# ignaschuemer7/soft-actor-critic

Measured on AMD Instinct MI355X. Metric: SAC gradient steps/sec + replay-sample GB/s, BipedalWalker batch=256, higher is better.
Workload: dtype fp32; 1 GPU; c2: BipedalWalker-v3 obs=24 act=4 2x[256, 256] MLPs, buffer=1000000, batch=256, auto-alpha, device sampler, fp32 arithmetic; global_batch=256, parallelism=replicas1, graph_chunk=64

## Files before the change

soft-actor-critic_amd/csrc/sac_split.h:

```cpp
#pragma once
#include "sac_phases.h"

#define SPLIT_H 256
#define SPLIT_HH 128
__host__ __device__ constexpr int split_wc(int elem_bytes) { return elem_bytes == 4 ? 4 : 2; }
__host__ __device__ constexpr int split_wcq(int elem_bytes) { return (void)elem_bytes, 4; }
__host__ __device__ constexpr int split_wpi(int elem_bytes) { return split_wc(elem_bytes); }
#define SPLIT_GP 4

enum SplitGran {
  GS_PI = 0,
  GS_PS = 1,
  GS_QT1 = 2,
  GS_QT2 = 3,
  GS_LP = 4,
  GS_QA1 = 5,
  GS_QA2 = 6,
  GS_C1 = 7,
  GS_C2 = 8,
  GS_COUNT = 9
};
__device__ __forceinline__ AS_G uint64_t* gs_at(const AS_C EngineDev& E, int kind, int rbi, int h) {
  return GP(uint64_t, E.gran2) + ((size_t)(kind * E.nrt + rbi) * SPLIT_GP + h) * E.gs2;
}

template <typename T, int NTW, int HC>
struct HTiles {
  typename MM<T>::Frag f[NTW][HC];
  float b[NTW];
};

template <typename T, int NTW, int HC, bool COH = false>
__device__ __forceinline__ void ht_issue(HTiles<T, NTW, HC>& ht, const GemmW& w) {
  constexpr uint32_t FSB = 64 * MM<T>::KL * sizeof(T);
  const int lane = threadIdx.x & 63, wave = wave_id();
  const int nch = w.cols / MM<T>::KC;
  const __amdgpu_buffer_rsrc_t rs = coh_rsrc(w.p, 0xFFFFFFF0u);
  static_for<NTW>([&](auto jc) {
    constexpr int j = decltype(jc)::value;
    int t = wave + j * SAC_NW;
    const bool has = t < w.NT;
    t = has ? t : w.NT - 1;
    const uint32_t o = (uint32_t)(((size_t)t * 16 * w.tcols + lane * MM<T>::KL) * sizeof(T));
    static_for<HC>([&](auto uc) {
      constexpr int u = decltype(uc)::value;
      const uint32_t cu = u < nch ? u : nch - 1;
      if (has)
        ht.f[j][u] = coh_frag<T, COH>(rs, o + cu * FSB);
      else
        ht.f[j][u] = typename MM<T>::Frag{};
    });
    if (w.bias) {
      const int n = t * 16 + (lane & 15);
      ht.b[j] = ldf<COH>(w.bias + (n < w.N ? n : w.N - 1));
    }
  });
}

template <typename T, int NTW, int HC, bool COH = false, typename Epi>
__device__ __forceinline__ void gemm_hs(const lf* __restrict__ A, int lda, const GemmW& w,
                                        const HTiles<T, NTW, HC>* ht, Epi&& epi) {
  typedef typename MM<T>::Frag F;
  constexpr int KC = MM<T>::KC, KL = MM<T>::KL;
  constexpr uint32_t FSB = 64 * KL * sizeof(T);
  const int lane = threadIdx.x & 63, wave = wave_id();
  const int c = lane & 15, g = lane >> 4;
  const int nch = w.cols / KC;
  const lf* arow = A + c * lda + g * KL;
  f32x4 acc[NTW][2];
  static_for<NTW>([&](auto jc) {
    constexpr int j = decltype(jc)::value;
    acc[j][0] = acc[j][1] = (f32x4){0.f, 0.f, 0.f, 0.f};
  });
  int ch0 = 0;
  if (ht) {
    F a[HC];
    static_for<HC>([&](auto uc) {
      constexpr int u = decltype(uc)::value;
      a[u] = MM<T>::from_lds(arow + (u < nch ? u : 0) * KC);
    });
    static_for<HC>([&](auto uc) {
      constexpr int u = decltype(uc)::value;
      if (u < nch)
        static_for<NTW>([&](auto jc) {
          constexpr int j = decltype(jc)::value;
          if (wave + j * SAC_NW < w.NT)
            MM<T>::mma(acc[j][u & 1], a[u], ht->f[j][u]);
        });
    });
    ch0 = HC;
  }
  if (ch0 < nch) {
    const __amdgpu_buffer_rsrc_t rs = coh_rsrc(w.p, 0xFFFFFFF0u);
    uint32_t o[NTW];
    static_for<NTW>([&](auto jc) {
      constexpr int j = decltype(jc)::value;
      int t = wave + j * SAC_NW;
      t = t < w.NT ? t : w.NT - 1;
      o[j] = (uint32_t)(((size_t)t * 16 * w.tcols + lane * KL) * sizeof(T));
    });
    for (int cb = ch0; cb < nch; cb += 8) {
      const int rem = nch - cb < 8 ? nch - cb : 8;
      F f[NTW][8], a[8];
      static_for<8>([&](auto uc) {
        constexpr int u = decltype(uc)::value;
        const uint32_t cu = cb + (u < rem ? u : rem - 1);
        static_for<NTW>([&](auto jc) {
          constexpr int j = decltype(jc)::value;
          f[j][u] = coh_frag<T, COH>(rs, o[j] + cu * FSB);
        });
      });
      static_for<8>([&](auto uc) {
        constexpr int u = decltype(uc)::value;
        a[u] = MM<T>::from_lds(arow + (cb + (u < rem ? u : rem - 1)) * KC);
      });
      static_for<8>([&](auto uc) {
        constexpr int u = decltype(uc)::value;
        if (u < rem)
          static_for<NTW>([&](auto jc) {
            constexpr int j = decltype(jc)::value;
            if (wave + j * SAC_NW < w.NT) MM<T>::mma(acc[j][u & 1], a[u], f[j][u]);
          });
      });
    }
  }
  static_for<NTW>([&](auto jc) {
    constexpr int j = decltype(jc)::value;
    const int t = wave + j * SAC_NW;
    if (t < w.NT) epi(j, t * 16 + c, acc[j][0] + acc[j][1]);
  });
}

#ifndef SAC_KS_HELD
#define SAC_KS_HELD 1
#endif
#ifndef SAC_KS_MAXC32
#define SAC_KS_MAXC32 1
#endif
#ifndef SAC_KS_C
#define SAC_KS_C 1
#endif
template <typename T, int MC = (sizeof(T) == 4 ? SAC_KS_MAXC32 : 1)>
struct KsHeld {
  static constexpr int MAXC = MC;
  typename MM<T>::Frag f[MAXC];
  bool ok;
};
template <typename T>
__device__ __forceinline__ void ks_slice(const GemmW& w, int& t, int& c0, int& c1, int& wpt) {
  const int wave = wave_id();
  const int NT = w.NT;
  wpt = SAC_NW / NT;
  t = wave % NT;
  const int sl = wave / NT;
  const int nch = w.cols / MM<T>::KC;
  const int per = (nch + wpt - 1) / wpt;
  c0 = sl * per;
  c1 = c0 + per < nch ? c0 + per : nch;
}
template <typename T, int MC, bool COH = false>
__device__ __forceinline__ void ks_issue(KsHeld<T, MC>& kh, const GemmW& w) {
  constexpr uint32_t FSB = 64 * MM<T>::KL * sizeof(T);
  int t, c0, c1, wpt;
  ks_slice<T>(w, t, c0, c1, wpt);
  const int nch = w.cols / MM<T>::KC, per = (nch + wpt - 1) / wpt;
  kh.ok = SAC_KS_HELD && per <= MC;
  if (!kh.ok) return;
  const __amdgpu_buffer_rsrc_t rs = coh_rsrc(w.p, 0xFFFFFFF0u);
  const uint32_t o = (uint32_t)(((size_t)t * 16 * w.tcols + (threadIdx.x & 63) * MM<T>::KL) * sizeof(T));
  static_for<MC>([&](auto uc) {
    constexpr int u = decltype(uc)::value;
    if (c0 + u < c1) kh.f[u] = coh_frag<T, COH>(rs, o + (c0 + u) * FSB);
  });
}

template <typename T, bool COH = false, int MC = 1>
__device__ __forceinline__ void gemm_ksplit(const lf* __restrict__ A, int lda, const GemmW& w, lf* red, lf* out,
                                            int ldo, const KsHeld<T, MC>* kh = nullptr) {
  typedef typename MM<T>::Frag F;
  constexpr int KC = MM<T>::KC, KL = MM<T>::KL;
  constexpr uint32_t FSB = 64 * KL * sizeof(T);
  const int lane = threadIdx.x & 63, wave = wave_id();
  const int c = lane & 15, g = lane >> 4;
  const int NT = w.NT;
  int t, c0, c1, wpt;
  ks_slice<T>(w, t, c0, c1, wpt);
  const __amdgpu_buffer_rsrc_t rs = coh_rsrc(w.p, 0xFFFFFFF0u);
  const uint32_t o = (uint32_t)(((size_t)t * 16 * w.tcols + lane * KL) * sizeof(T));
  const lf* arow = A + c * lda + g * KL;
  f32x4 acc = {0.f, 0.f, 0.f, 0.f};
  if (kh && kh->ok) {
    static_for<MC>([&](auto uc) {
      constexpr int u = decltype(uc)::value;
      if (c0 + u < c1) MM<T>::mma(acc, MM<T>::from_lds(arow + (c0 + u) * KC), kh->f[u]);
    });
    c1 = c0;
  }
  for (int cb = c0; cb < c1; cb += 4) {
    const int rem = c1 - cb < 4 ? c1 - cb : 4;
    F f[4], a[4];
    static_for<4>([&](auto uc) {
      constexpr int u = decltype(uc)::value;
      const int cu = cb + (u < rem ? u : rem - 1);
      f[u] = coh_frag<T, COH>(rs, o + cu * FSB);
      a[u] = MM<T>::from_lds(arow + cu * KC);
    });
    static_for<4>([&](auto uc) {
      constexpr int u = decltype(uc)::value;
      if (u < rem) MM<T>::mma(acc, a[u], f[u]);
    });
  }
#pragma unroll
  for (int i = 0; i < 4; ++i) red[wave * 256 + (g * 4 + i) * 16 + c] = acc[i];
  __syncthreads();
  for (int i = threadIdx.x; i < 256 * NT; i += SAC_THREADS) {
    const int tt = i / 256, e = i % 256, r = e / 16, cc = e % 16;
    float s = 0.f;
    for (int q = 0; q < wpt; ++q) s += red[(q * NT + tt) * 256 + e];
    out[r * ldo + tt * 16 + cc] = s;
  }
  __syncthreads();
}

template <typename T>
__device__ __forceinline__ void target_critic_split_body(const EngineDev* __restrict__ Ep, const sac_replay& rb,
                                                         const int32_t* __restrict__ inj_idx_,
                                                         const float* __restrict__ inj_eps_, int bidA,
                                                         const StepCtx& sc) {
  const AS_C EngineDev& E = *(const AS_C EngineDev*)Ep;
  extern __shared__ float lds_raw[];
  lf* lds = (lf*)lds_raw;
  constexpr int R = SAC_ROWS, HH = SPLIT_HH;
  constexpr int KC = MM<T>::KC;
  constexpr int HC0 = 64 / KC;
  constexpr int NCH_H = SPLIT_H / KC;
  constexpr int NCH_HH = HH / KC;
  const int tid = threadIdx.x;
  constexpr int WP = split_wpi(sizeof(T));
  const int n2 = 2 * E.nrt, n0 = WP * E.nrt;
  const int grp = bidA < n0 ? 0 : 1 + (bidA - n0) / n2;
  const int idx = bidA < n0 ? bidA : (bidA - n0) % n2;
  const int h = bidA < n0 ? idx % WP : idx & 1, rbi = bidA < n0 ? idx / WP : idx >> 1;
  const int HHr = grp == 0 ? SPLIT_H / WP : SPLIT_HH;
  const int role = grp;
  const bool is_pi = role == 0 || role == 5;
  const int ni = is_pi ? NET_PI : role <= 2 ? NET_Q1T + role - 1 : NET_Q1 + role - 3;
  const AS_C NetDev& net = E.net[ni];
  const AS_C LayerDev& L0 = net.l[0];
  const AS_C LayerDev& L1 = net.l[1];
  const AS_C LayerDev& L2 = net.l[2];
  STAMP(0);
  const GemmW w0 = gw_fwd(L0);
  const GemmW w1 = gw_sub<T>(L1.Wc, L1.Kp, h * HHr, HHr, 0, L1.Kp, L1.bias + h * HHr, HHr);
  HTiles<T, 2, HC0> h0;
  HTiles<T, 1, NCH_H> h1;
  ht_issue<T, 2, HC0>(h0, w0);

  const int B = E.B, Bp = E.Bp, O = E.O, A = E.A, ld = E.ld, ldo = E.ldo;
  const int r0 = rbi * R;
  const int nvalid = min(R, B - r0);
  const uint32_t ep = sc.ep;
  const AS_G int32_t* inj_idx = GPC(int32_t, inj_idx_);
  const AS_G float* inj_eps = GPC(float, inj_eps_);
  lf* Xb = lds + E.o_X;
  lf* H0 = lds + E.o_Y;
  lf* P0 = lds + E.o_P1[0];
  lf* P1 = lds + E.o_P1[1];
  lf* H1 = lds + E.o_P2[0];
  lf* U1 = lds + E.o_P2[1];
  const int ldp0 = E.ldp1[0], ldp1 = E.ldp1[1], ldh1 = E.ldp2[0], ldu1 = E.ldp2[1];
  lf* outB = lds + E.o_out;
  lf* red = lds + E.o_red;
  lf* sB = lds + E.o_s;
  lf* s2B = lds + E.o_s2;
  lf* aB = lds + E.o_a;
  lf* a2B = lds + E.o_a2;
  lf* rB = lds + E.o_r;
  lf* dB = lds + E.o_d;
  lf* epsB = lds + E.o_et;
  lf* lpB = lds + E.o_lp;
  AS_L int64_t* slotB = (AS_L int64_t*)(lds + E.o_slot);
  AS_G float* stats = GP(float, E.stats);

  const uint64_t step = sc.step;
  const int par = sc.par;
#ifndef SAC_ADAM_LAST
#define SAC_ADAM_LAST 1
#endif
  const bool adam_blk = (SAC_ADAM_LAST ? (role == 5 && rbi == E.nrt - 1 && h == 1) : (role == 0 && rbi == 0 && h == 0));
  if (adam_blk && tid < 4 && (tid < 3 || (E.auto_entropy && E.alpha_update))) {
    const double t = GP(double, E.opt_steps)[tid] + 1.0;
    GP(double, E.opt_steps)[tid] = t;
    if (tid < 3) {
      const double lr = tid == 0 ? E.actor_lr : E.critic_lr;
      GP(float, E.adam_sc)[par * 6 + tid * 2] = (float)(-(lr / (1.0 - pow((double)E.beta1, t))));
      GP(float, E.adam_sc)[par * 6 + tid * 2 + 1] = (float)sqrt(1.0 - pow((double)E.beta2, t));
    } else {
      GP(double, E.alpha_sc)[par * 2] = 1.0 - pow((double)E.beta1, t);
      GP(double, E.alpha_sc)[par * 2 + 1] = 1.0 - pow((double)E.beta2, t);
    }
  }
  const int64_t rb_size = GPC(int64_t, rb.state)[0], rb_pos = GPC(int64_t, rb.state)[1];
  bool staged = false;
  bool h1_issued = false;
  if (E.stage && !inj_idx) {
    const AS_G float* rec = GPC(float, E.stg) + stage_rec(E, step, rbi);
    const AS_C uint64_t* hdr = (const AS_C uint64_t*)rec;
    const AS_G float* p = rec + 16;
    constexpr int NS = (R * 32 + SAC_THREADS - 1) / SAC_THREADS;
    if (O <= 32) {
      float rs[2][NS], ra[NS], rr = 0.f, rd = 0.f;
#pragma unroll
      for (int u = 0; u < NS; ++u) {
        const int i = tid + u * SAC_THREADS;
        rs[0][u] = i < R * O ? p[i] : 0.f;
        rs[1][u] = i < R * O ? p[R * O + i] : 0.f;
        ra[u] = i < R * A ? p[2 * R * O + i] : 0.f;
      }
      if (tid < R) {
        rr = p[2 * R * O + R * A + tid];
        rd = p[2 * R * O + R * A + R + tid];
      }
      ht_issue<T, 1, NCH_H>(h1, w1);
      h1_issued = true;
#pragma unroll
      for (int u = 0; u < NS; ++u) {
        const int i = tid + u * SAC_THREADS;
        if (i < R * O) {
          sB[i] = rs[0][u];
          s2B[i] = rs[1][u];
        }
        if (i < R * A) aB[i] = ra[u];
      }
      if (tid < R) {
        rB[tid] = rr;
        dB[tid] = rd;
      }
      STAMP(22);
    } else {
      for (int i = tid; i < R * O; i += SAC_THREADS) {
        sB[i] = p[i];
        s2B[i] = p[R * O + i];
      }
      for (int i = tid; i < R * A; i += SAC_THREADS) aB[i] = p[2 * R * O + i];
      if (tid < R) {
        rB[tid] = p[2 * R * O + R * A + tid];
        dB[tid] = p[2 * R * O + R * A + R + tid];
      }
    }
    staged = hdr[0] == step && hdr[1] == (uint64_t)rb_size && hdr[2] == (uint64_t)rb_pos &&
             hdr[3] == (uint64_t)(uintptr_t)rb.obs && hdr[4] == (uint64_t)GPC(int64_t, rb.state)[2];
  }
  if (!h1_issued) ht_issue<T, 1, NCH_H>(h1, w1);
  GemmW w2n = gw_sub<T>(L2.Wc, L2.Kp, 0, L2.Np, h * HHr, HHr, nullptr, 0);
  w2n.NT = (L2.N + 15) >> 4;
  KsHeld<T> kh2;
  kh2.ok = false;
  if (sizeof(T) == 2) ks_issue<T>(kh2, w2n);
  if (staged && rbi == 0 && role == 0 && h == 0 && tid == 0)
    *(AS_G uint64_t*)(GP(uint32_t, E.sync) + 4) = step;
  if (!staged) {
    tile_slots(E, rb, step, rb_size, rb_pos, r0, inj_idx, slotB);
    __syncthreads();
    gather_rows<lf*>(rb, slotB, O, A, sB, s2B, aB, rB, dB);
  }
  if (role == 1 || role == 2 || role == 5) {
    const int which = role == 5 ? 1 : 0;
    const int NP = (A + 1) / 2;
    for (int i = tid; i < R * NP; i += SAC_THREADS) {
      const int r = i / NP, pp = i % NP, b = r0 + r;
      float e0 = 0.f, e1 = 0.f;
      if (b < B) {
        if (inj_eps) {
          e0 = inj_eps[((size_t)which * B + b) * A + 2 * pp];
          if (2 * pp + 1 < A) e1 = inj_eps[((size_t)which * B + b) * A + 2 * pp + 1];
        } else {
          philox_normal2(E.seed, step, (uint32_t)b, (uint32_t)which, (uint32_t)pp, e0, e1);
        }
      }
      epsB[r * A + 2 * pp] = e0;
      if (2 * pp + 1 < A) epsB[r * A + 2 * pp + 1] = e1;
    }
  }
  __syncthreads();
  STAMP(1);

  auto head = [&](const AS_G uint64_t* g0, const AS_G uint64_t* g1, bool tgt, lf* actB, lf* lpOut, bool stash) {
    const AS_C NetDev& pn = E.net[NET_PI];
    const float* b2 = pn.l[2].bias;
    const int AP = A <= 1 ? 1 : 1 << (32 - __builtin_clz(A - 1));
    const int rpp = SAC_THREADS / AP;
    const int jj = tid % AP;
    const float b2mu = jj < A ? ldf<false>(b2 + jj) : 0.f, b2ls = jj < A ? ldf<false>(b2 + A + jj) : 0.f;
    for (int base = 0; base < R; base += rpp) {
      const int r = base + tid / AP, j = jj;
      const bool live = r < R && j < A;
      float lp = 0.f, corr = 0.f;
      if (live) {
        float mu, lsr;
        if (tgt) {
          const AS_G uint64_t* gg[2 * WP];
#pragma unroll
          for (int p = 0; p < WP; ++p) {
            gg[p] = g0 + (size_t)p * E.gs2 + r * 2 * A + j;
            gg[WP + p] = g0 + (size_t)p * E.gs2 + r * 2 * A + A + j;
          }
          float v[2 * WP];
          gran_getn<2 * WP>(E, gg, ep, v);
          float smu = v[0], sls = v[WP];
#pragma unroll
          for (int p = 1; p < WP; ++p) {
            smu += v[p];
            sls += v[WP + p];
          }
          mu = smu + b2mu;
          lsr = sls + b2ls;
        } else {
          const float pown0 = outB[r * ldo + j], pown1 = outB[r * ldo + A + j];
          const AS_G uint64_t* gg[2] = {g1 + r * 2 * A + j, g1 + r * 2 * A + A + j};
          float v[2];
          gran_getn<2>(E, gg, ep, v);
          const float ppe0 = v[0], ppe1 = v[1];
          mu = (h == 0 ? pown0 + ppe0 : ppe0 + pown0) + b2mu;
          lsr = (h == 0 ? pown1 + ppe1 : ppe1 + pown1) + b2ls;
        }
        const float e = epsB[r * A + j];
        const float lo = E.ls_min, hi = E.ls_max;
        const float ls = lsr < lo ? lo : (lsr > hi ? hi : lsr);
        const float sd = expf(ls);
        const float z = mu + e * sd;
        const float act_v = tanhf(z) * E.scale;
        const float diff = z - mu;
        const float var = sd * sd;
        lp = -(diff * diff) / (2.f * var) - logf(sd) - HALF_LOG_2PI;
        corr = 2.f * ((LOG2F - z) - softplus20(-2.f * z));
        actB[r * A + j] = act_v;
        if (stash) {
          const int b = r0 + r;
          float* hs = E.head_st + (size_t)b * 4 * A;
          st_f<false>(hs + j, mu);
          st_f<false>(hs + A + j, lsr);
          st_f<false>(hs + 2 * A + j, z);
          st_f<false>(hs + 3 * A + j, e);
          st_f<false>(E.a_st + (size_t)b * A + j, act_v);
        }
      }
      for (int o = 1; o < AP; o <<= 1) {
        lp += __shfl_xor(lp, o, 64);
        corr += __shfl_xor(corr, o, 64);
      }
      if (live && j == 0) lpOut[r] = lp - corr;
    }
    __syncthreads();
  };

  auto no_hook = [] {};
  auto forward01 = [&](bool keepP, bool stXT, bool pi_actor, auto&& after_l1, bool l0_done = false) {
    const int act = net.hid_act;
    if (!l0_done) gemm_hs<T, 2, HC0, false>(Xb, ld, w0, &h0, [&](int j, int col, const f32x4& acc) {
      const bool nv = col < L0.N;
      const float bn = h0.b[j];
#pragma unroll
      for (int i = 0; i < 4; ++i) {
        const int r = (((threadIdx.x & 63) >> 4) << 2) + i;
        const float p = nv ? acc[i] + bn : 0.f;
        if (keepP) P0[r * ldp0 + col] = p;
        H0[r * ld + col] = act == ACT_RELU ? (p > 0.f ? p : 0.f) : p;
      }
    });
    if (!l0_done) {
      if (act != ACT_RELU && act != ACT_ID) act_pass_fwd<R>(H0, ld, L0.Np >> 4, act);
      __syncthreads();
    }
    if (pi_actor && h == 0 && act != ACT_RELU) {
      float* ps = L0.pstash + (size_t)r0 * L0.Np;
      for (int i = tid; i < R * L0.Np; i += SAC_THREADS) st_f<false>(ps + i, P0[(i / L0.Np) * ldp0 + i % L0.Np]);
    }
    if (stXT && h == 0)
      store_T<T, R>(H0, ld, L1.Kp, L1.K, (T*)L1.XT + (pi_actor ? par * L1.xt_par : 0), Bp, r0, nvalid, nullptr);
    STAMP(2);
    if (sizeof(T) == 4 && !kh2.ok) ks_issue<T, KsHeld<T>::MAXC, false>(kh2, w2n);
    gemm_hs<T, 1, NCH_H, false>(H0, ld, w1, &h1, [&](int j, int col, const f32x4& acc) {
      const float bn = h1.b[j];
#pragma unroll
      for (int i = 0; i < 4; ++i) {
        const int r = (((threadIdx.x & 63) >> 4) << 2) + i;
        const float p = acc[i] + bn;
        if (keepP) P1[r * ldp1 + col] = p;
        H1[r * ldh1 + col] = act == ACT_RELU ? (p > 0.f ? p : 0.f) : p;
      }
    });
    after_l1();
    if (act != ACT_RELU && act != ACT_ID) act_pass_fwd<R>(H1, ldh1, HHr >> 4, act);
    __syncthreads();
    if (pi_actor && act != ACT_RELU) {
      float* ps = L1.pstash + (size_t)r0 * L1.Np + h * HH;
      for (int i = tid; i < R * HH; i += SAC_THREADS) st_f<false>(ps + (i / HH) * L1.Np + i % HH, P1[(i / HH) * ldp1 + i % HH]);
    }
    if (stXT)
      store_T<T, R>(H1, ldh1, HH, HH, (T*)L2.XT + (pi_actor ? par * L2.xt_par : 0) + (size_t)h * HH * Bp, Bp, r0,
                       nvalid, nullptr);
    STAMP(3);
    gemm_ksplit<T, false, decltype(kh2)::MAXC>(H1, ldh1, w2n, red, outB, ldo, &kh2);
    STAMP(4);
  };

  auto build_x = [&](const lf* st, const lf* ac, int na) {
    const int Kp0 = L0.Kp;
    for (int i = tid; i < R * Kp0; i += SAC_THREADS) {
      const int r = i / Kp0, k = i % Kp0;
      Xb[r * ld + k] = k < O ? st[r * O + k] : (k < O + na ? ac[r * A + (k - O)] : 0.f);
    }
    __syncthreads();
  };

  const float alpha32 = (float)*GPC(double, E.alpha_state + 1);
  if (role == 0) {
    build_x(s2B, aB, 0);
    forward01(false, false, false, no_hook);
    AS_G uint64_t* g = gs_at(E, GS_PI, rbi, h);
    for (int i = tid; i < R * 2 * A; i += SAC_THREADS) gran_put(g + i, outB[(i / (2 * A)) * ldo + i % (2 * A)], ep);
    STAMP(6);
  } else if (role == 5) {
    if (h == 0)
      for (int i = tid; i < R * O; i += SAC_THREADS) st_f<false>(E.s_st + (size_t)r0 * O + i, sB[i]);
    build_x(sB, aB, 0);
    store_T<T, R>(Xb, ld, L0.Kp, L0.K, (T*)L0.XT + par * L0.xt_par, 2 * Bp, h * Bp + r0, nvalid, nullptr);
    forward01(true, true, true, no_hook);
    AS_G uint64_t* g = gs_at(E, GS_PS, rbi, h);
    for (int i = tid; i < R * 2 * A; i += SAC_THREADS) gran_put(g + i, outB[(i / (2 * A)) * ldo + i % (2 * A)], ep);
    head(nullptr, gs_at(E, GS_PS, rbi, 1 - h), false, a2B, lpB, h == 0);
    if (h == 0 && tid < nvalid) {
      const int b = r0 + tid;
      st_f<false>(E.lp_st + par * E.Br + b, lpB[tid]);
      stats[4 + B + b] = lpB[tid];
    }
    STAMP(6);
  } else if (role == 1 || role == 2) {
    const int t = role - 1;
    if (sizeof(T) == 4) ks_issue<T, KsHeld<T>::MAXC, false>(kh2, w2n);
    const int Kp0 = L0.Kp, nch0 = Kp0 / KC;
    const bool early0 = nch0 <= HC0;
    if (early0) {
      build_x(s2B, a2B, 0);
      const int cs = O / KC, cb = (O + KC - 1) / KC;
      const int lane = tid & 63, wave = wave_id(), c = lane & 15, g = lane >> 4;
      const lf* arow = Xb + c * ld + g * MM<T>::KL;
      f32x4 acc[2][2];
#pragma unroll
      for (int j = 0; j < 2; ++j) acc[j][0] = acc[j][1] = (f32x4){0.f, 0.f, 0.f, 0.f};
      auto chunks = [&](int c0, int c1) __attribute__((always_inline)) {
        static_for<HC0>([&](auto uc) {
          constexpr int u = decltype(uc)::value;
          if (u >= c0 && u < c1) {
            const typename MM<T>::Frag a = MM<T>::from_lds(arow + u * KC);
            static_for<2>([&](auto jc) {
              constexpr int j = decltype(jc)::value;
              if (wave + j * SAC_NW < w0.NT) MM<T>::mma(acc[j][u & 1], a, h0.f[j][u]);
            });
          }
        });
      };
      chunks(0, cb);
      __syncthreads();
      if (cb > cs)
        for (int i = tid; i < R * KC; i += SAC_THREADS) {
          const int r = i / KC, k = cs * KC + i % KC;
          if (k < O) Xb[r * ld + k] = 0.f;
        }
      head(gs_at(E, GS_PI, rbi, 0), nullptr, true, a2B, lpB, false);
      if (t == 0 && h == 0 && tid < R) gran_put(gs_at(E, GS_LP, rbi, 0) + tid, lpB[tid], ep);
      STAMP(7);
      for (int i = tid; i < R * A; i += SAC_THREADS) Xb[(i / A) * ld + O + i % A] = a2B[i];
      __syncthreads();
      chunks(cs, nch0);
      const int act = net.hid_act;
      static_for<2>([&](auto jc) {
        constexpr int j = decltype(jc)::value;
        const int tt = wave + j * SAC_NW;
        if (tt < w0.NT) {
          const int col = tt * 16 + c;
          const bool nv = col < L0.N;
          const f32x4 sum = acc[j][0] + acc[j][1];
#pragma unroll
          for (int i = 0; i < 4; ++i) {
            const float p = nv ? sum[i] + h0.b[j] : 0.f;
            H0[(g * 4 + i) * ld + col] = act == ACT_RELU ? (p > 0.f ? p : 0.f) : p;
          }
        }
      });
      if (act != ACT_RELU && act != ACT_ID) act_pass_fwd<R>(H0, ld, L0.Np >> 4, act);
      __syncthreads();
      forward01(false, false, false, no_hook, true);
    } else {
      head(gs_at(E, GS_PI, rbi, 0), nullptr, true, a2B, lpB, false);
      if (t == 0 && h == 0 && tid < R) gran_put(gs_at(E, GS_LP, rbi, 0) + tid, lpB[tid], ep);
      STAMP(7);
      build_x(s2B, a2B, A);
      forward01(false, false, false, no_hook);
    }
    if (tid < R) gran_put(gs_at(E, t ? GS_QT2 : GS_QT1, rbi, h) + tid, outB[tid * ldo], ep);
    STAMP(9);
    if (t == 0 && h == 0 && tid < 64) {
      float sq[2] = {0.f, 0.f};
      if (tid < R) {
        const int b = r0 + tid;
        const bool v = tid < nvalid;
        const AS_C NetDev& t1 = E.net[NET_Q1T];
        const AS_C NetDev& t2 = E.net[NET_Q2T];
        const float bt1 = ldf<false>(t1.l[2].bias), bt2 = ldf<false>(t2.l[2].bias);
        const float bq[2] = {ldf<false>(E.net[NET_Q1].l[2].bias), ldf<false>(E.net[NET_Q2].l[2].bias)};
        const AS_G uint64_t* gg[7] = {gs_at(E, GS_QT1, rbi, 1) + tid, gs_at(E, GS_QT2, rbi, 0) + tid,
                                      gs_at(E, GS_QT2, rbi, 1) + tid, gs_at(E, GS_QA1, rbi, 0) + tid,
                                      gs_at(E, GS_QA1, rbi, 1) + tid, gs_at(E, GS_QA2, rbi, 0) + tid,
                                      gs_at(E, GS_QA2, rbi, 1) + tid};
        float gv[7];
        gran_getn<7>(E, gg, ep, gv);
        const float q1tp = outB[tid * ldo] + gv[0] + bt1;
        const float q2tp = gv[1] + gv[2] + bt2;
        const float q1t = t1.out_act == ACT_ID ? q1tp : act_fwd(t1.out_act, q1tp);
        const float q2t = t2.out_act == ACT_ID ? q2tp : act_fwd(t2.out_act, q2tp);
        const float y = rB[tid] + (E.gamma * (1.f - dB[tid])) * (fmin_nan(q1t, q2t) - alpha32 * lpB[tid]);
        if (b < B) stats[4 + b] = y;
#pragma unroll
        for (int qi = 0; qi < 2; ++qi) {
          const AS_C NetDev& qn = E.net[NET_Q1 + qi];
          const float qpre = (gv[3 + 2 * qi] + gv[4 + 2 * qi]) + bq[qi];
          const float q = qn.out_act == ACT_ID ? qpre : act_fwd(qn.out_act, qpre);
          const float d = q - y;
          sq[qi] = v ? d * d : 0.f;
          float seed = v ? (2.0f / (float)B) * d : 0.f;
          if (qn.out_act != ACT_ID) seed = act_bwd(qn.out_act, qpre, seed);
          st_f<false>(E.seedq + qi * Bp + b, seed);
        }
      }
#pragma unroll
      for (int qi = 0; qi < 2; ++qi) {
        const float s2 = wave_sum(sq[qi]);
        if (tid == 0) st_f<false>(E.lossp + (par * E.nrt + rbi) * 4 + qi, s2);
      }
    }
  } else {
    const int qi = role - 3;
    const GemmW wt1 = gw_sub<T>(L1.WTc, L1.Np, 0, L1.Kp, h * HH, HH, nullptr, 0);
    HTiles<T, 2, NCH_HH> ht1;
    if constexpr (sizeof(T) == 2) ht_issue<T, 2, NCH_HH, false>(ht1, wt1);
    static_assert(SAC_THREADS % SPLIT_HH == 0, "one W2 column per thread in the unit-seed loop");
    const float w2n = ldf<false>(net.P + L2.w_off + h * HH + tid % HH);
    build_x(sB, aB, A);
    if (qi == 0) store_T<T, R>(Xb, ld, L0.Kp, L0.K, L0.XT, 2 * Bp, h * Bp + r0, nvalid, nullptr);
    forward01(true, true, false, [&] {
      if constexpr (sizeof(T) == 4) ht_issue<T, 2, NCH_HH, false>(ht1, wt1);
    });
    if (tid < R) gran_put(gs_at(E, qi ? GS_QA2 : GS_QA1, rbi, h) + tid, outB[tid * ldo], ep);
    {
      for (int i = tid; i < R * HH; i += SAC_THREADS) {
        const int r = i / HH, n = i % HH;
        U1[r * ldu1 + n] = act_bwd(net.hid_act, P1[r * ldp1 + n], w2n);
      }
      __syncthreads();
      gemm_hs<T, 2, NCH_HH, false>(U1, ldu1, wt1, &ht1, [&](int j, int col, const f32x4& acc) {
        const bool kv = col < L1.K;
#pragma unroll
        for (int i = 0; i < 4; ++i) {
          const int r = (((threadIdx.x & 63) >> 4) << 2) + i;
          float v = kv ? acc[i] : 0.f;
          if (net.hid_act == ACT_RELU && !(P0[r * ldp0 + col] > 0.f)) v = 0.f;
          Xb[r * ld + col] = v;
        }
      });
      if (net.hid_act != ACT_RELU && net.hid_act != ACT_ID)
        act_pass_bwd<R>(Xb, ld, P0, ldp0, L1.Kp >> 4, L1.K, net.hid_act);
      __syncthreads();
    }
    STAMP(16);
    store_T<T, R>(U1, ldu1, HH, HH, (T*)L1.GT + (size_t)h * HH * Bp, Bp, r0, nvalid, nullptr);
    store_T<T, R>(Xb, ld, L0.Np, L0.N, L0.GT, 2 * Bp, h * Bp + r0, nvalid, nullptr);
    if (h == 0) {
      lf* g2 = outB;
      for (int i = tid; i < R * 32; i += SAC_THREADS) g2[(i / 32) * ldo + i % 32] = (i % 32) == 0 ? 1.f : 0.f;
      __syncthreads();
      store_T<T, R>(g2, ldo, L2.Np, L2.N, L2.GT, Bp, r0, nvalid, nullptr);
    }
    STAMP(15);
    STAMP(11 + 2 * qi);
  }
}

template <typename T>
__global__ void __launch_bounds__(SAC_THREADS) sac_target_critic_split(const EngineDev* __restrict__ Ep, sac_replay rb,
                                                                        const int32_t* __restrict__ inj_idx_,
                                                                        const float* __restrict__ inj_eps_) {
#ifdef SAC_STAMPS
  const long long t_entry = __builtin_amdgcn_s_memrealtime();
#endif
  PREFETCH_ARG(Ep);
  const AS_C EngineDev& E0 = *(const AS_C EngineDev*)Ep;
  const uint64_t step = *GPC(uint64_t, E0.rng_step);
  const StepCtx sc{step, *GPC(uint32_t, E0.sync) + 1u, (int)(step & 1)};
#ifdef SAC_STAMPS
  if (threadIdx.x == 0 && E0.stamps) {
    GP(long long, E0.stamps)[blockIdx.x * 64 + 20] = t_entry;
    GP(long long, E0.stamps)[blockIdx.x * 64 + 21 + (step == ~0ull ? 1 : 0)] = __builtin_amdgcn_s_memrealtime();
  }
#endif
  int bidA = (int)blockIdx.x;
  if (E0.role_xcd) {
    constexpr int WP = split_wpi(sizeof(T));
    const int nrt = E0.nrt, n0 = WP * nrt, n2 = 2 * nrt;
    const int u = (bidA % 8) * ((int)gridDim.x / 8) + bidA / 8;
    if (u < n0) {
      bidA = (u % nrt) * WP + u / nrt;
    } else {
      const int v = u - n0, w = v % n2;
      bidA = n0 + (v / n2) * n2 + (w % nrt) * 2 + w / nrt;
    }
  }
  target_critic_split_body<T>(Ep, rb, inj_idx_, inj_eps_, bidA, sc);
  const AS_C EngineDev& E = *(const AS_C EngineDev*)Ep;
  (void)E;
  END_STAMP(60);
}

template <typename T>
__device__ __forceinline__ void actor_split_body(const EngineDev* __restrict__ Ep, int bid, const StepCtx& sc) {
  const AS_C EngineDev& E = *(const AS_C EngineDev*)Ep;
  extern __shared__ float lds_raw[];
  lf* lds = (lf*)lds_raw;
  constexpr int R = SAC_ROWS, WQ = split_wcq(sizeof(T)), WP = split_wc(sizeof(T));
  constexpr int HQ = SPLIT_H / WQ, HH = SPLIT_H / WP;
  constexpr int KC = MM<T>::KC;
  constexpr int HC0 = 64 / KC;
  constexpr int NCH_H = SPLIT_H / KC;
  constexpr int NCH_HH = HH / KC, NCH_HQ = HQ / KC;
  constexpr int NCH_32 = 32 / KC;
  const int tid = threadIdx.x;
  const int nq = WQ * E.nrt;
  const bool is_pi = bid >= 2 * nq;
  const int qi = is_pi ? 0 : bid / nq;
  const int idx = is_pi ? bid - 2 * nq : bid % nq;
  const int h = is_pi ? idx % WP : idx % WQ, rbi = is_pi ? idx / WP : idx / WQ;
  STAMP(32);
  const int B = E.B, Bp = E.Bp, O = E.O, A = E.A, ld = E.ld, ldo = E.ldo;
  const int r0 = rbi * R;
  const int nvalid = min(R, B - r0);
  const uint32_t ep = sc.ep;
  const int par = sc.par;
  lf* Xb = lds + E.o_X;
  lf* H0 = lds + E.o_Y;
  lf* P0 = lds + E.o_P1[0];
  lf* P1 = lds + E.o_P1[1];
  lf* H1 = lds + E.o_P2[0];
  lf* U1 = lds + E.o_P2[1];
  const int ldp0 = E.ldp1[0], ldp1 = E.ldp1[1], ldh1 = E.ldp2[0], ldu1 = E.ldp2[1];
  lf* outB = lds + E.o_out;
  lf* red = lds + E.o_red;
  lf* sB = lds + E.o_s;
  lf* aB = lds + E.o_a;
  lf* lpB = lds + E.o_lp;
  lf* gaB = lds + E.o_ga;
  lf* goutB = lds + E.o_gout;
  lf* g1B = lds + E.o_g;
  lf* g2B = lds + E.o_g2;
  const float alpha32 = (float)*GPC(double, E.alpha_state + 1);

  if (!is_pi) {
    const AS_C NetDev& net = E.net[NET_Q1 + qi];
    const AS_C LayerDev& L0 = net.l[0];
    const AS_C LayerDev& L1 = net.l[1];
    const AS_C LayerDev& L2 = net.l[2];
    const GemmW w0 = gw_fwd(L0);
    const GemmW w1 = gw_sub<T>(L1.Wc, L1.Kp, h * HQ, HQ, 0, L1.Kp, L1.bias + h * HQ, HQ);
    HTiles<T, 2, HC0> h0;
    HTiles<T, 1, NCH_H> h1;
    const GemmW wt1 = gw_sub<T>(L1.WTc, L1.Np, 0, L1.Kp, h * HQ, HQ, nullptr, 0);
    HTiles<T, 2, NCH_HQ> ht1;
    ht_issue<T, 2, HC0>(h0, w0);
    ht_issue<T, 1, NCH_H>(h1, w1);
    ht_issue<T, 2, NCH_HQ>(ht1, wt1);
    GemmW w2 = gw_sub<T>(L2.Wc, L2.Kp, 0, L2.Np, h * HQ, HQ, nullptr, 0);
    w2.NT = (L2.N + 15) >> 4;
    const int k0 = (O >> 4) << 4, k1 = (O + A + 15) >> 4 << 4;
    GemmW wt0 = gw_sub<T>(L0.WTc, L0.Np, k0, k1 - k0, 0, L0.Np, nullptr, 0);
    KsHeld<T, sizeof(T) == 4 ? 2 : 1> kc2;
    KsHeld<T, sizeof(T) == 4 ? 8 : 1> kc0;
    kc2.ok = kc0.ok = false;
    static_assert(SAC_THREADS % HQ == 0, "one W2 column per thread in the unit-seed loop");
    const float w2n = GPC(float, net.P + L2.w_off)[h * HQ + tid % HQ];
    for (int i = tid; i < R * O; i += SAC_THREADS) sB[i] = GPC(float, E.s_st)[(size_t)r0 * O + i];
    for (int i = tid; i < R * A; i += SAC_THREADS) aB[i] = GPC(float, E.a_st)[(size_t)r0 * A + i];
    if (SAC_KS_C) {
      ks_issue<T, decltype(kc2)::MAXC>(kc2, w2);
      if (sizeof(T) == 2) ks_issue<T, decltype(kc0)::MAXC>(kc0, wt0);
    }
    __syncthreads();
    const int Kp0 = L0.Kp;
    for (int i = tid; i < R * Kp0; i += SAC_THREADS) {
      const int r = i / Kp0, k = i % Kp0;
      Xb[r * ld + k] = k < O ? sB[r * O + k] : (k < O + A ? aB[r * A + (k - O)] : 0.f);
    }
    __syncthreads();
    STAMP(33);
    const int act = net.hid_act;
    gemm_hs<T, 2, HC0, false>(Xb, ld, w0, &h0, [&](int j, int col, const f32x4& acc) {
      const bool nv = col < L0.N;
      const float bn = h0.b[j];
#pragma unroll
      for (int i = 0; i < 4; ++i) {
        const int r = (((threadIdx.x & 63) >> 4) << 2) + i;
        const float p = nv ? acc[i] + bn : 0.f;
        P0[r * ldp0 + col] = p;
        H0[r * ld + col] = act == ACT_RELU ? (p > 0.f ? p : 0.f) : p;
      }
    });
    if (act != ACT_RELU && act != ACT_ID) act_pass_fwd<R>(H0, ld, L0.Np >> 4, act);
    __syncthreads();
    gemm_hs<T, 1, NCH_H, false>(H0, ld, w1, &h1, [&](int j, int col, const f32x4& acc) {
      const float bn = h1.b[j];
#pragma unroll
      for (int i = 0; i < 4; ++i) {
        const int r = (((threadIdx.x & 63) >> 4) << 2) + i;
        const float p = acc[i] + bn;
        P1[r * ldp1 + col] = p;
        H1[r * ldh1 + col] = act == ACT_RELU ? (p > 0.f ? p : 0.f) : p;
      }
    });
    if (SAC_KS_C && sizeof(T) == 4) ks_issue<T, decltype(kc0)::MAXC>(kc0, wt0);
    if (act != ACT_RELU && act != ACT_ID) act_pass_fwd<R>(H1, ldh1, HQ >> 4, act);
    __syncthreads();
    gemm_ksplit<T, false, decltype(kc2)::MAXC>(H1, ldh1, w2, red, outB, ldo, &kc2);
    STAMP(36 + qi);
    {
      for (int i = tid; i < R * HQ; i += SAC_THREADS) {
        const int r = i / HQ, n = i % HQ;
        U1[r * ldu1 + n] = act_bwd(act, P1[r * ldp1 + n], w2n);
      }
      __syncthreads();
      gemm_hs<T, 2, NCH_HQ, false>(U1, ldu1, wt1, &ht1, [&](int j, int col, const f32x4& acc) {
        const bool kv = col < L1.K;
#pragma unroll
        for (int i = 0; i < 4; ++i) {
          const int r = (((threadIdx.x & 63) >> 4) << 2) + i;
          float v = kv ? acc[i] : 0.f;
          if (act == ACT_RELU && !(P0[r * ldp0 + col] > 0.f)) v = 0.f;
          Xb[r * ld + col] = v;
        }
      });
      if (act != ACT_RELU && act != ACT_ID) act_pass_bwd<R>(Xb, ld, P0, ldp0, L1.Kp >> 4, L1.K, act);
      __syncthreads();
      gemm_ksplit<T, false, decltype(kc0)::MAXC>(Xb, ld, wt0, red, H0, ld, &kc0);
      AS_G uint64_t* g = gs_at(E, GS_C1 + qi, rbi, h);
      for (int i = tid; i < R * A; i += SAC_THREADS) gran_put(g + i, H0[(i / A) * ld + (O - k0) + i % A], ep);
      if (tid < R) gran_put(g + R * A + tid, outB[tid * ldo], ep);
    }
    STAMP(38 + qi);
    return;
  }

  const AS_C NetDev& pi = E.net[NET_PI];
  const AS_C LayerDev& L0 = pi.l[0];
  const AS_C LayerDev& L1 = pi.l[1];
  const AS_C LayerDev& L2 = pi.l[2];
  const GemmW wt2 = gw_sub<T>(L2.WTc, L2.Np, h * HH, HH, 0, L2.Np, nullptr, 0);
  const GemmW wt1 = gw_sub<T>(L1.WTc, L1.Np, 0, L1.Kp, h * HH, HH, nullptr, 0);
  HTiles<T, 1, NCH_32> ht2;
  HTiles<T, 2, NCH_HH> ht1;
  ht_issue<T, 1, NCH_32, false>(ht2, wt2);
  ht_issue<T, 2, NCH_HH, false>(ht1, wt1);
  {
    if (pi.hid_act == ACT_RELU) {
      const AS_G T* x1 = GPC(T, L1.XT) + par * L1.xt_par + r0;
      for (int i = tid; i < R * L0.Np; i += SAC_THREADS) {
        const int k = i / R, r = i % R;
        P0[r * ldp0 + k] = k < L1.K ? (float)x1[(size_t)k * Bp + r] : 0.f;
      }
      const AS_G T* x2 = GPC(T, L2.XT) + par * L2.xt_par + (size_t)h * HH * Bp + r0;
      for (int i = tid; i < R * HH; i += SAC_THREADS) {
        const int k = i / R, r = i % R;
        P1[r * ldp1 + k] = (float)x2[(size_t)k * Bp + r];
      }
    } else {
      const float* p0 = L0.pstash + (size_t)r0 * L0.Np;
      for (int i = tid; i < R * L0.Np; i += SAC_THREADS) P0[(i / L0.Np) * ldp0 + i % L0.Np] = ldf<false>(p0 + i);
      const float* p1 = L1.pstash + (size_t)r0 * L1.Np + h * HH;
      for (int i = tid; i < R * HH; i += SAC_THREADS)
        P1[(i / HH) * ldp1 + i % HH] = ldf<false>(p1 + (i / HH) * L1.Np + i % HH);
    }
    if (tid < R) lpB[tid] = ldf<false>(E.lp_st + par * E.Br + r0 + tid);
  }
  float hsv[4] = {0.f, 0.f, 0.f, 0.f};
  if (tid < R * A && r0 + tid / A < E.Br) {
    const float* hs = E.head_st + (size_t)(r0 + tid / A) * 4 * A;
#pragma unroll
    for (int q = 0; q < 4; ++q) hsv[q] = ldf<false>(hs + q * A + tid % A);
  }
  const float bq1 = ldf<false>(E.net[NET_Q1].l[2].bias), bq2 = ldf<false>(E.net[NET_Q2].l[2].bias);
  __syncthreads();
  STAMP(34);
  const AS_G uint64_t* c1p[WQ];
  const AS_G uint64_t* c2p[WQ];
#pragma unroll
  for (int p = 0; p < WQ; ++p) {
    c1p[p] = gs_at(E, GS_C1, rbi, p);
    c2p[p] = gs_at(E, GS_C2, rbi, p);
  }
  if (R * A <= 64) {
    if (tid < 64) {
      const bool live = tid < R * A;
      const int i = live ? tid : 0, r = i / A, rq = tid < R ? tid : 0;
      const AS_G uint64_t* gg[4 * WQ];
#pragma unroll
      for (int p = 0; p < WQ; ++p) {
        gg[p] = c1p[p] + i;
        gg[WQ + p] = c2p[p] + i;
        gg[2 * WQ + p] = c1p[p] + R * A + rq;
        gg[3 * WQ + p] = c2p[p] + R * A + rq;
      }
      float gv[4 * WQ];
      gran_getn1<4 * WQ>(E, gg, ep, gv);
      float term = 0.f, w1 = 0.f, w2 = 0.f;
      if (tid < R) {
        const bool v = tid < nvalid;
        const AS_C NetDev& q1n = E.net[NET_Q1];
        const AS_C NetDev& q2n = E.net[NET_Q2];
        float q1p = gv[2 * WQ], q2p = gv[3 * WQ];
#pragma unroll
        for (int p = 1; p < WQ; ++p) {
          q1p += gv[2 * WQ + p];
          q2p += gv[3 * WQ + p];
        }
        q1p += bq1;
        q2p += bq2;
        const float q1 = q1n.out_act == ACT_ID ? q1p : act_fwd(q1n.out_act, q1p);
        const float q2 = q2n.out_act == ACT_ID ? q2p : act_fwd(q2n.out_act, q2p);
        const float m = fmin_nan(q1, q2);
        term = v ? alpha32 * lpB[tid] - m : 0.f;
        const float gm = v ? -1.0f / (float)B : 0.f;
        w1 = (q1 == q2) ? gm * 0.5f : (q1 > q2 ? 0.f : gm);
        w2 = (q1 == q2) ? gm * 0.5f : (q1 < q2 ? 0.f : gm);
        if (q1n.out_act != ACT_ID) w1 = act_bwd(q1n.out_act, q1p, w1);
        if (q2n.out_act != ACT_ID) w2 = act_bwd(q2n.out_act, q2p, w2);
      }
      term = wave_sum(term);
      if (tid == 0 && h == 0) st_f<false>(E.lossp + (par * E.nrt + rbi) * 4 + 2, term);
      const float w1r = __shfl(w1, r, 64), w2r = __shfl(w2, r, 64);
      if (live) {
        float da1 = gv[0], da2 = gv[WQ];
#pragma unroll
        for (int p = 1; p < WQ; ++p) {
          da1 += gv[p];
          da2 += gv[WQ + p];
        }
        gaB[i] = w1r * da1 + w2r * da2;
      }
    }
    __syncthreads();
  } else {
  if (tid < 64) {
    float term = 0.f;
    if (tid < R) {
      const bool v = tid < nvalid;
      const AS_C NetDev& q1n = E.net[NET_Q1];
      const AS_C NetDev& q2n = E.net[NET_Q2];
      const AS_G uint64_t* gg[2 * WQ];
#pragma unroll
      for (int p = 0; p < WQ; ++p) {
        gg[p] = c1p[p] + R * A + tid;
        gg[WQ + p] = c2p[p] + R * A + tid;
      }
      float gv[2 * WQ];
      gran_getn<2 * WQ>(E, gg, ep, gv);
      float q1p = gv[0], q2p = gv[WQ];
#pragma unroll
      for (int p = 1; p < WQ; ++p) {
        q1p += gv[p];
        q2p += gv[WQ + p];
      }
      q1p += bq1;
      q2p += bq2;
      const float q1 = q1n.out_act == ACT_ID ? q1p : act_fwd(q1n.out_act, q1p);
      const float q2 = q2n.out_act == ACT_ID ? q2p : act_fwd(q2n.out_act, q2p);
      const float m = fmin_nan(q1, q2);
      term = v ? alpha32 * lpB[tid] - m : 0.f;
      const float gm = v ? -1.0f / (float)B : 0.f;
      float w1 = (q1 == q2) ? gm * 0.5f : (q1 > q2 ? 0.f : gm);
      float w2 = (q1 == q2) ? gm * 0.5f : (q1 < q2 ? 0.f : gm);
      if (q1n.out_act != ACT_ID) w1 = act_bwd(q1n.out_act, q1p, w1);
      if (q2n.out_act != ACT_ID) w2 = act_bwd(q2n.out_act, q2p, w2);
      g1B[tid] = w1;
      g2B[tid] = w2;
    }
    term = wave_sum(term);
    if (tid == 0 && h == 0) st_f<false>(E.lossp + (par * E.nrt + rbi) * 4 + 2, term);
  }
  __syncthreads();
  for (int i = tid; i < R * A; i += SAC_THREADS) {
    const int r = i / A;
    const AS_G uint64_t* gg[2 * WQ];
#pragma unroll
    for (int p = 0; p < WQ; ++p) {
      gg[p] = c1p[p] + i;
      gg[WQ + p] = c2p[p] + i;
    }
    float gv[2 * WQ];
    gran_getn<2 * WQ>(E, gg, ep, gv);
    float da1 = gv[0], da2 = gv[WQ];
#pragma unroll
    for (int p = 1; p < WQ; ++p) {
      da1 += gv[p];
      da2 += gv[WQ + p];
    }
    gaB[i] = g1B[r] * da1 + g2B[r] * da2;
  }
  __syncthreads();
  }
  STAMP(39);
  static_assert(SAC_ROWS * 32 <= SAC_THREADS, "one (row, action dim) per thread");
  if (tid < R * A) {
    const int i = tid;
    const int r = i / A, j = i % A;
    const bool v = r < nvalid;
    const float gl = v ? alpha32 * (1.0f / (float)B) : 0.f;
    const float lo = E.ls_min, hi = E.ls_max, scale = E.scale;
    const float mu = hsv[0], lsr = hsv[1], z = hsv[2], e = hsv[3];
    const float ls = lsr < lo ? lo : (lsr > hi ? hi : lsr);
    const float sd = expf(ls);
    const float t = tanhf(z);
    const float diff = z - mu, var = sd * sd;
    float g_z = (gaB[r * A + j] * scale) * (1.f - t * t);
    g_z = g_z + (-gl) * 2.f * (-1.f + 2.f * softplus20_grad(-2.f * z));
    const float two_var = 2.f * var;
    const float g_sq = -gl / two_var;
    const float g_twovar = gl * (diff * diff) / (two_var * two_var);
    const float g_var = 2.f * g_twovar;
    float g_std = 2.f * sd * g_var - gl / sd;
    const float g_diff = 2.f * diff * g_sq;
    g_z = g_z + g_diff;
    const float g_mu = -g_diff + g_z;
    g_std = g_std + g_z * e;
    const float g_ls = g_std * sd;
    const bool in_range = (lsr >= lo) && (lsr <= hi);
    goutB[r * ldo + j] = v ? g_mu : 0.f;
    goutB[r * ldo + A + j] = (v && in_range) ? g_ls : 0.f;
  }
  {
    const int NOp = L2.Np, pad = NOp - 2 * A;
    for (int i = tid; i < R * pad; i += SAC_THREADS) goutB[(i / pad) * ldo + 2 * A + i % pad] = 0.f;
  }
  __syncthreads();
  if (h == 0) store_T<T, R>(goutB, ldo, L2.Np, L2.N, L2.GT, Bp, r0, nvalid, L2.dbp);
  const int act = pi.hid_act;
  gemm_hs<T, 1, NCH_32, false>(goutB, ldo, wt2, &ht2, [&](int j, int col, const f32x4& acc) {
#pragma unroll
    for (int i = 0; i < 4; ++i) {
      const int r = (((threadIdx.x & 63) >> 4) << 2) + i;
      float v = acc[i];
      if (act == ACT_RELU && !(P1[r * ldp1 + col] > 0.f)) v = 0.f;
      U1[r * ldu1 + col] = v;
    }
  });
  if (act != ACT_RELU && act != ACT_ID) act_pass_bwd<R>(U1, ldu1, P1, ldp1, HH >> 4, HH, act);
  __syncthreads();
  store_T<T, R>(U1, ldu1, HH, HH, (T*)L1.GT + (size_t)h * HH * Bp, Bp, r0, nvalid, L1.dbp ? L1.dbp + h * HH : nullptr, nullptr, L1.N);
  gemm_hs<T, 2, NCH_HH, false>(U1, ldu1, wt1, &ht1, [&](int j, int col, const f32x4& acc) {
    const bool kv = col < L1.K;
#pragma unroll
    for (int i = 0; i < 4; ++i) {
      const int r = (((threadIdx.x & 63) >> 4) << 2) + i;
      float v = kv ? acc[i] : 0.f;
      if (act == ACT_RELU && !(P0[r * ldp0 + col] > 0.f)) v = 0.f;
      Xb[r * ld + col] = v;
    }
  });
  if (act != ACT_RELU && act != ACT_ID) act_pass_bwd<R>(Xb, ld, P0, ldp0, L1.Kp >> 4, L1.K, act);
  __syncthreads();
  store_T<T, R>(Xb, ld, L0.Np, L0.N, L0.GT, WP * Bp, h * Bp + r0, nvalid, L0.dbp);
  STAMP(35);
}

template <typename T>
__global__ void __launch_bounds__(SAC_THREADS) sac_actor_split(const EngineDev* __restrict__ Ep, sac_replay rb) {
  PREFETCH_ARG(Ep);
  const AS_C EngineDev& E = *(const AS_C EngineDev*)Ep;
  extern __shared__ float lds_raw[];
  const int bid = (int)blockIdx.x;
  const int nrole = (2 * split_wcq(sizeof(T)) + split_wc(sizeof(T))) * E.nrt;
  if (bid >= nrole) {
    stage_next_batch(E, rb, bid - nrole, (lf*)lds_raw, *GPC(uint64_t, E.rng_step));
  } else {
    const uint64_t step = *GPC(uint64_t, E.rng_step);
    actor_split_body<T>(Ep, bid, StepCtx{step, *GPC(uint32_t, E.sync) + 1u, (int)(step & 1)});
  }
  phase_c_done(E);
  END_STAMP(61);
}
```

Before: 19910 gradient steps/s.

## Fuse narrow Q-head output into hidden-layer epilogue and hoist actor-head math

For fp32 critics with a single-output last layer and ReLU/identity activations, the last-layer dot product is folded into the layer-1 GEMM epilogue. It uses a 16-lane shuffle reduction and a small cross-wave sum, replacing the separate k-split GEMM and the H1 staging writes. Small input tiles are loaded straight into registers and written to the X buffer, which removes one staging pass and one barrier. The actor-head gradient terms that do not depend on the critic gradients, and the zeroing of the padding, are moved ahead of the gradient gather so they overlap with it. Both paths sit behind compile-time flags, at the cost of extra register use and more code paths.

```diff
diff --git a/soft-actor-critic_amd/csrc/sac_split.h b/soft-actor-critic_amd/csrc/sac_split.h
--- a/soft-actor-critic_amd/csrc/sac_split.h
+++ b/soft-actor-critic_amd/csrc/sac_split.h
@@ -222,6 +222,26 @@
   __syncthreads();
 }
 
+#ifndef SAC_NARROW_FUSED
+#define SAC_NARROW_FUSED 1
+#endif
+#ifndef SAC_NARROW_SMALL
+#define SAC_NARROW_SMALL 1
+#endif
+
+__device__ __forceinline__ float rows16_sum(const float (&p)[4]) {
+  const int c = threadIdx.x & 15;
+  const bool b3 = c & 8, b2 = c & 4;
+  const float m0 = b3 ? p[2] : p[0], o0 = b3 ? p[0] : p[2];
+  const float m1 = b3 ? p[3] : p[1], o1 = b3 ? p[1] : p[3];
+  const float q0 = m0 + __shfl_xor(o0, 8, 64), q1 = m1 + __shfl_xor(o1, 8, 64);
+  const float m = b2 ? q1 : q0, o = b2 ? q0 : q1;
+  float v = m + __shfl_xor(o, 4, 64);
+  v += __shfl_xor(v, 1, 64);
+  v += __shfl_xor(v, 2, 64);
+  return v;
+}
+
 template <typename T>
 __device__ __forceinline__ void target_critic_split_body(const EngineDev* __restrict__ Ep, const sac_replay& rb,
                                                          const int32_t* __restrict__ inj_idx_,
@@ -787,21 +807,38 @@
     kc2.ok = kc0.ok = false;
     static_assert(SAC_THREADS % HQ == 0, "one W2 column per thread in the unit-seed loop");
     const float w2n = GPC(float, net.P + L2.w_off)[h * HQ + tid % HQ];
-    for (int i = tid; i < R * O; i += SAC_THREADS) sB[i] = GPC(float, E.s_st)[(size_t)r0 * O + i];
-    for (int i = tid; i < R * A; i += SAC_THREADS) aB[i] = GPC(float, E.a_st)[(size_t)r0 * A + i];
+    const int act = net.hid_act;
+    const int Kp0 = L0.Kp;
+    const bool relu_id = act == ACT_RELU || act == ACT_ID;
+    const bool fuse2 = SAC_NARROW_FUSED && sizeof(T) == 4 && L2.N == 1 && relu_id;
+    const int lane = tid & 63, wv = wave_id();
+    float w2l = 0.f;
+    const bool x_direct = SAC_NARROW_SMALL && R * Kp0 <= SAC_THREADS;
+    float xv = 0.f;
+    if (x_direct) {
+      const int r = tid / Kp0, k = tid % Kp0;
+      if (tid < R * Kp0 && k < O + A)
+        xv = k < O ? GPC(float, E.s_st)[(size_t)r0 * O + r * O + k] : GPC(float, E.a_st)[(size_t)r0 * A + r * A + (k - O)];
+    } else {
+      for (int i = tid; i < R * O; i += SAC_THREADS) sB[i] = GPC(float, E.s_st)[(size_t)r0 * O + i];
+      for (int i = tid; i < R * A; i += SAC_THREADS) aB[i] = GPC(float, E.a_st)[(size_t)r0 * A + i];
+    }
+    if (fuse2) w2l = GPC(float, net.P + L2.w_off)[h * HQ + (wv < w1.NT ? wv : 0) * 16 + (lane & 15)];
     if (SAC_KS_C) {
-      ks_issue<T, decltype(kc2)::MAXC>(kc2, w2);
+      if (!fuse2) ks_issue<T, decltype(kc2)::MAXC>(kc2, w2);
       if (sizeof(T) == 2) ks_issue<T, decltype(kc0)::MAXC>(kc0, wt0);
     }
-    __syncthreads();
-    const int Kp0 = L0.Kp;
-    for (int i = tid; i < R * Kp0; i += SAC_THREADS) {
-      const int r = i / Kp0, k = i % Kp0;
-      Xb[r * ld + k] = k < O ? sB[r * O + k] : (k < O + A ? aB[r * A + (k - O)] : 0.f);
+    if (x_direct) {
+      if (tid < R * Kp0) Xb[(tid / Kp0) * ld + tid % Kp0] = xv;
+    } else {
+      __syncthreads();
+      for (int i = tid; i < R * Kp0; i += SAC_THREADS) {
+        const int r = i / Kp0, k = i % Kp0;
+        Xb[r * ld + k] = k < O ? sB[r * O + k] : (k < O + A ? aB[r * A + (k - O)] : 0.f);
+      }
     }
     __syncthreads();
     STAMP(33);
-    const int act = net.hid_act;
     gemm_hs<T, 2, HC0, false>(Xb, ld, w0, &h0, [&](int j, int col, const f32x4& acc) {
       const bool nv = col < L0.N;
       const float bn = h0.b[j];
@@ -817,18 +854,33 @@
     __syncthreads();
     gemm_hs<T, 1, NCH_H, false>(H0, ld, w1, &h1, [&](int j, int col, const f32x4& acc) {
       const float bn = h1.b[j];
+      float q2[4];
 #pragma unroll
       for (int i = 0; i < 4; ++i) {
         const int r = (((threadIdx.x & 63) >> 4) << 2) + i;
         const float p = acc[i] + bn;
+        const float hv = act == ACT_RELU ? (p > 0.f ? p : 0.f) : p;
         P1[r * ldp1 + col] = p;
-        H1[r * ldh1 + col] = act == ACT_RELU ? (p > 0.f ? p : 0.f) : p;
+        if (!fuse2) H1[r * ldh1 + col] = hv;
+        q2[i] = hv * w2l;
+      }
+      if (fuse2) {
+        const float s2 = rows16_sum(q2);
+        if ((lane & 3) == 0) red[wv * R + ((lane >> 4) << 2) + ((lane & 15) >> 2)] = s2;
       }
     });
     if (SAC_KS_C && sizeof(T) == 4) ks_issue<T, decltype(kc0)::MAXC>(kc0, wt0);
     if (act != ACT_RELU && act != ACT_ID) act_pass_fwd<R>(H1, ldh1, HQ >> 4, act);
     __syncthreads();
-    gemm_ksplit<T, false, decltype(kc2)::MAXC>(H1, ldh1, w2, red, outB, ldo, &kc2);
+    if (fuse2) {
+      if (tid < R) {
+        float s = red[tid];
+        for (int w = 1; w < w1.NT && w < SAC_NW; ++w) s += red[w * R + tid];
+        outB[tid * ldo] = s;
+      }
+    } else {
+      gemm_ksplit<T, false, decltype(kc2)::MAXC>(H1, ldh1, w2, red, outB, ldo, &kc2);
+    }
     STAMP(36 + qi);
     {
       for (int i = tid; i < R * HQ; i += SAC_THREADS) {
@@ -895,6 +947,30 @@
     for (int q = 0; q < 4; ++q) hsv[q] = ldf<false>(hs + q * A + tid % A);
   }
   const float bq1 = ldf<false>(E.net[NET_Q1].l[2].bias), bq2 = ldf<false>(E.net[NET_Q2].l[2].bias);
+  float hb_omt = 0.f, hb_sp = 0.f, hb_gstd = 0.f, hb_gdiff = 0.f, hb_sd = 0.f;
+  if (SAC_NARROW_SMALL) {
+    if (tid < R * A) {
+      const bool v = tid / A < nvalid;
+      const float gl = v ? alpha32 * (1.0f / (float)B) : 0.f;
+      const float lo = E.ls_min, hi = E.ls_max;
+      const float mu = hsv[0], lsr = hsv[1], z = hsv[2];
+      const float ls = lsr < lo ? lo : (lsr > hi ? hi : lsr);
+      const float sd = expf(ls);
+      const float t = tanhf(z);
+      const float diff = z - mu, var = sd * sd;
+      hb_omt = 1.f - t * t;
+      hb_sp = (-gl) * 2.f * (-1.f + 2.f * softplus20_grad(-2.f * z));
+      const float two_var = 2.f * var;
+      const float g_sq = -gl / two_var;
+      const float g_twovar = gl * (diff * diff) / (two_var * two_var);
+      const float g_var = 2.f * g_twovar;
+      hb_gstd = 2.f * sd * g_var - gl / sd;
+      hb_gdiff = 2.f * diff * g_sq;
+      hb_sd = sd;
+    }
+    const int NOp = L2.Np, pad = NOp - 2 * A;
+    for (int i = tid; i < R * pad; i += SAC_THREADS) goutB[(i / pad) * ldo + 2 * A + i % pad] = 0.f;
+  }
   __syncthreads();
   STAMP(34);
   const AS_G uint64_t* c1p[WQ];
@@ -1016,7 +1092,23 @@
   }
   STAMP(39);
   static_assert(SAC_ROWS * 32 <= SAC_THREADS, "one (row, action dim) per thread");
-  if (tid < R * A) {
+  if (SAC_NARROW_SMALL) {
+    if (tid < R * A) {
+      const int r = tid / A, j = tid % A;
+      const bool v = r < nvalid;
+      const float lo = E.ls_min, hi = E.ls_max, scale = E.scale;
+      const float lsr = hsv[1], e = hsv[3];
+      float g_z = (gaB[r * A + j] * scale) * hb_omt;
+      g_z = g_z + hb_sp;
+      g_z = g_z + hb_gdiff;
+      const float g_mu = -hb_gdiff + g_z;
+      const float g_std = hb_gstd + g_z * e;
+      const float g_ls = g_std * hb_sd;
+      const bool in_range = (lsr >= lo) && (lsr <= hi);
+      goutB[r * ldo + j] = v ? g_mu : 0.f;
+      goutB[r * ldo + A + j] = (v && in_range) ? g_ls : 0.f;
+    }
+  } else if (tid < R * A) {
     const int i = tid;
     const int r = i / A, j = i % A;
     const bool v = r < nvalid;
@@ -1043,7 +1135,7 @@
     goutB[r * ldo + j] = v ? g_mu : 0.f;
     goutB[r * ldo + A + j] = (v && in_range) ? g_ls : 0.f;
   }
-  {
+  if (!SAC_NARROW_SMALL) {
     const int NOp = L2.Np, pad = NOp - 2 * A;
     for (int i = tid; i < R * pad; i += SAC_THREADS) goutB[(i / pad) * ldo + 2 * A + i % pad] = 0.f;
   }
```

Measured after the change: 20410 gradient steps/s (median of 6 runs). 2.5% higher.
